# datasciencetoolkit/NextGP.jl

Measured on AMD Instinct MI355X. Metric: gibbs_iterations_per_sec, higher is better.
Workload: dtype f64; 1 GPU; single-trait Gibbs sweep, N=50000 individuals x P=600000 SNPs, marker sets BayesPR(200000) + BayesPR(200000) + BayesPR(200000), fp32 panel in HBM (BASELINE.json configs[3]: multi-breed random regression = three BayesPR marker sets of 200,000 SNPs); N=50000, P=600000, chains=1, panel_dtype=f32, accumulate_dtype=f64

## Files before the change

nextgp.jl_amd/csrc/ngp_api.hip:

```cpp
#include <hip/hip_runtime.h>

#include <dlfcn.h>

#include <algorithm>
#include <chrono>
#include <cmath>
#include <cstdio>
#include <cstdlib>
#include <condition_variable>
#include <cstddef>
#include <cstring>
#include <deque>
#include <memory>
#include <mutex>
#include <queue>
#include <string>
#include <thread>
#include <vector>

#include "../../include/nextgp_hip.h"
#include "ngp_kernels.h"
#include "ngp_random.h"
#include "ngp_dense.h"
#include "ngp_logvar.h"
// ... 25 lines not shown
    T *p = nullptr;
    PinnedArray() = default;
    PinnedArray(const PinnedArray &) = delete;
    PinnedArray &operator=(const PinnedArray &) = delete;
    PinnedArray(PinnedArray &&o) noexcept : p(o.p) { o.p = nullptr; }
    PinnedArray &operator=(PinnedArray &&o) noexcept { if (this != &o) { reset(); p = o.p; o.p = nullptr; } return *this; }
    ~PinnedArray() { reset(); }
    void reset() { if (p) { (void)hipHostFree(p); p = nullptr; } }
    hipError_t alloc_raw(size_t n) { reset(); const hipError_t e = hipHostMalloc((void **)&p, n * sizeof(T), hipHostMallocDefault); if (e != hipSuccess) p = nullptr; return e; }
    T *get() const { return p; }
    operator T *() const { return p; }
};

struct FileCloser {
    void operator()(FILE *f) const { std::fclose(f); }
};
using File = std::unique_ptr<FILE, FileCloser>;

struct HFix {
    int64_t ncol = 0, off = 0;
    DevArray<double> d_X, d_xpx0, d_xpxR, d_lhs0, d_rhs0;
};

struct DenseK {
    DevArray<double> K;
    int64_t q = 0, ld = 0;
    uint64_t digest = 0;
};

struct Grm {
    std::shared_ptr<DenseK> m;
    int state = 0, method = 1;
    int64_t N = 0, ncols = 0;
    double sum2pq = 0.0;
};

struct HRand {
    int64_t q = 0;
    double df = 0.0, scale = 0.0, varU0 = 0.0;
    bool offdiag = false;
    uint64_t fine_calls = 0;
    DevArray<long long> d_lptr, d_kptr;
    DevArray<int> d_lrows, d_level, d_kcol;
    DevArray<double> d_kval, d_kdiag, d_zpz;
    DevArray<double> d_u, d_sum_u;
    DevArray<double> d_vu;
    DevArray<double> d_scr;
    uint64_t sig = 0;
    std::shared_ptr<DenseK> dk;
    struct Launch { int wide; int d0, d1; long long r0, r1; };
    DevArray<int> d_order;
    DevArray<long long> d_dptr;
    std::vector<Launch> plan;
    int64_t ndepth = 0;
    int sched_mode = 0;
    bool scheduled() const { return sched_mode == 2 || (sched_mode == 0 && q > NGP_RS_AUTO_LEVELS_PER_DEPTH * ndepth); }
};

struct HLv {
    int set = -1;
    int64_t n = 0;
    int ncov = 0, mode = 0;
    double frac = 0.0, varZeta0 = 0.0;
    std::vector<double> zeta0;
    DevArray<double> d_C, d_iCpC, d_zeta, d_logv, d_part, d_vpart;
    DevArray<double> d_st;
    DevArray<int> d_trapseg;
};

struct PanelMem {
    DevArray<float> tiles;
    DevArray<double> mean;
    DevArray<double> gramx, mpm;
    double mpm_max = 0.0;
};

struct SampleStream {
    static constexpr int NSLOT = 4;
    File f;
    std::string path;
    size_t rec_bytes = 0;
    bool header_written = false;
    int device = 0;
    DevArray<unsigned char> d_slot[NSLOT];
    PinnedArray<unsigned char> h_slot[NSLOT];
    hipEvent_t ev_packed[NSLOT] = {nullptr, nullptr, nullptr, nullptr}, ev_copied[NSLOT] = {nullptr, nullptr, nullptr, nullptr};
    hipStream_t copy_stream = nullptr;
    std::thread writer;
    std::mutex mu;
    std::condition_variable cv;
    std::deque<int> queue;
    bool busy[NSLOT] = {false, false, false, false};
    bool stop = false, io_error = false;
    int64_t nenq = 0, nwritten = 0, ndropped = 0;
    ~SampleStream();
};

struct HSet {
    int64_t col0, ncol;
    int method;
    double df, scale;
    int64_t nreg;
    int64_t vb_off;
    int estPi;
    uint64_t fine_calls;
    double pi0;
    std::vector<double> vb0;
    int K = 0;
    std::vector<double> vcls, rpi;
    int tk = 0;
    int64_t nloc = 0;
    int lv = -1;
};

std::string g_create_err;


struct PlanRequest {
    int storage = 0;
    int mode = 1;
    int lag = 8;
    bool lag_auto = true;
    int near_req = 0;
    int max_shards_req = 0;
    int streamer_req = 0;
};

struct SweepPlan {
    int mode = 1;
    int64_t R = 0, S = 0;
    int V = 1;
    int D = 1;
    int NG = 1;
    int near = 3;
    int streamer = 1;
    int nchain = 8;
};

constexpr size_t NGP_LDS_MAX = 160 * 1024;

void choose_layout(int64_t N, int64_t max_shards, int64_t r_cap, int64_t *R, int64_t *S, bool prefer_odd = true) {
    int64_t r0 = (N + max_shards - 1) / max_shards;
    int64_t m = (r0 + 3) / 4;
    if (m < 1) m = 1;
    if (prefer_odd && (m & 1) == 0 && 4 * (m + 1) <= r_cap) m += 1;
    int64_t r = 4 * m;
    if (r > r_cap) r = r_cap;
    *R = r;
    *S = (N + r - 1) / r;
}

size_t sampler_lds(SweepKernel k) {
    const size_t base = (size_t)(3 * 4096 + 2 * NGP_RING * NGP_BLK + 6 * NGP_BLK) * sizeof(double) + 2 * NGP_BLK * sizeof(int) + 320;
    if (k == SweepKernel::lean) return base;
    if (k == SweepKernel::r || k == SweepKernel::multi_r) return base + NGP_SAMPLER_TUPLE_LDS + NGP_SAMPLER_R_LDS;
    return base + NGP_SAMPLER_TUPLE_LDS;
}

size_t streamer_lds(const SweepPlan &p, int K) {
    const int R = (int)p.R;
    if (K > 1) return p.streamer == 3 ? ngp_rows_multi_lds_bytes(R, K, true) : (p.streamer == 2 ? ngp_rows_multi_lds_bytes(R, K) : ngp_multi_lds_bytes(R, K));
    if (p.streamer >= 2) {
        const size_t nq = (p.streamer == 3) ? (size_t)R / 16 : (size_t)R / 4, hq = std::min<size_t>(NGP_ROWS_HMAX, (nq + 1) / 2);
        return (2 * nq + hq) * NGP_QS + (size_t)p.V * ((R + 7) & ~7) * 8 + 2 * NGP_ROWS_NW * NGP_BLK * 8 + 2 * NGP_DLS * 8 + 16 * 8 + 64 + 1024;
    }
    return 2 * (size_t)(R / 4) * NGP_QS + (size_t)R * 16 + 4096 + 2 * 512 + 128 + 3072 + (size_t)R * 64;
}

size_t sweep_lds(const SweepPlan &p, SweepKernel k, int K = 1) {
    const size_t streamer = streamer_lds(p, K);
    size_t lds = std::max(streamer, sampler_lds(k));
    if (K == 1 && streamer + 8192 <= NGP_LDS_MAX) lds = std::max(lds, streamer + 8192);
    return lds;
}

int fused_pair(const SweepPlan &p, int K) { return (p.streamer == 1 && K >= NGP_PAIR_FROM) ? 1 : 0; }

int64_t sweep_grid(const SweepPlan &p, int K = 1) { return K + ngp_multi_reducers(K, p.NG, fused_pair(p, K)) + p.S / p.V; }

SweepKernel pick_kernel(const SweepPlan &p, int K, bool diag, bool tup, bool rset) {
    if (K > 1) {
        if (rset && sweep_lds(p, SweepKernel::multi_r, K) <= NGP_LDS_MAX) return SweepKernel::multi_r;
        return tup ? SweepKernel::multi_tup : SweepKernel::multi;
    }
    if (p.V > 1) return SweepKernel::tall;
    if (diag) return SweepKernel::diag;
    if (rset && sweep_lds(p, SweepKernel::r) <= NGP_LDS_MAX) return SweepKernel::r;
    if (tup || rset) return SweepKernel::tup;
    return SweepKernel::lean;
}

const void *sweep_kernel(SweepKernel k) {
    for (auto unit : {sweep_kernel_0, sweep_kernel_1, sweep_kernel_2, sweep_kernel_3})
        if (const void *f = unit(k)) return f;
    return nullptr;
}

void launch_sweep_kernel(SweepKernel k, int64_t grid, size_t lds, hipStream_t stream, void *args) {
    void *a[] = {args};
    (void)hipLaunchKernel(sweep_kernel(k), dim3((unsigned)grid), dim3(NGP_WG), a, lds, stream);
}

int plan_sweep(int64_t N, int cu_count, const PlanRequest &q, SweepPlan *out, const char **msg) {
    SweepPlan p;
    p.mode = q.mode;
    int64_t max_shards = cu_count - 1 - (cu_count + NGP_GRP - 1) / NGP_GRP;
    if (q.max_shards_req > 0) max_shards = std::min<int64_t>(max_shards, q.max_shards_req);
    if (q.storage == 1) {
        if (q.mode != 1) { *msg = "compact storage runs in the persistent sweep (ngp_configure mode 1) only"; return NGP_ERR_ARG; }
        const int64_t r0 = (N + max_shards - 1) / max_shards;
        p.R = 16 * std::max<int64_t>(1, (r0 + 15) / 16);
        if (p.R > NGP_U8_MAX_R) { *msg = "N too large for one resident wave of streamers in compact storage"; return NGP_ERR_ARG; }
        p.S = (N + p.R - 1) / p.R;
        p.streamer = 3;
        p.nchain = NGP_ROWS_NW;
        const int nt = ngp_u8_tasks((int)p.R);
        const int want = q.lag_auto ? 8 : q.lag;
        if (nt == 1) p.D = want >= 12 ? 12 : (want >= 8 ? 8 : (want >= 6 ? 6 : (want >= 4 ? 4 : 3)));
        else if (nt == 2) p.D = want >= 8 ? 8 : 4;
        else p.D = 4;
        p.near = q.near_req ? q.near_req : ((p.R > 128) ? 2 : 3);
    } else {
        if (p.mode == 1) {
            int tallV = 0;
            int64_t w_max = 0;
            for (int v = 2; v <= 3 && !tallV; v++) {
                if (q.streamer_req != 0 && q.streamer_req != 2 * v) continue;
                if (q.streamer_req == 0 && N <= max_shards * 256) continue;
                SweepPlan t;
                t.V = v;
                auto fits = [&](int64_t w) { t.S = v * w; t.NG = (int)((t.S + NGP_GRP - 1) / NGP_GRP); return sweep_grid(t) <= cu_count; };
                int64_t w = cu_count - 1;
                while (w > 1 && !fits(w)) w--;
                if (q.max_shards_req > 0) w = std::max<int64_t>(1, std::min<int64_t>(w, q.max_shards_req / v));
                if (N <= v * w * NGP_ROWS_MAX_R && q.lag >= 3) { tallV = v; w_max = w; }
            }
            if (tallV) {
                choose_layout(N, tallV * w_max, NGP_ROWS_MAX_R, &p.R, &p.S, q.max_shards_req <= 0);
                p.S = (p.S + tallV - 1) / tallV * tallV;
                p.V = tallV;
            } else if (N > max_shards * 256) p.mode = 0;
            else choose_layout(N, max_shards, 256, &p.R, &p.S, q.max_shards_req <= 0);
        }
        if (p.mode == 0) choose_layout(N, 256, 508, &p.R, &p.S);
        p.D = (p.mode == 1) ? std::min(q.lag, 8) : 1;
        if (p.mode == 1 && p.R <= NGP_ROWS_MAX_R && q.lag >= 3 && (q.streamer_req == 2 || (q.streamer_req == 0 && p.R >= 64))) p.streamer = 2;
        if (p.V > 1) p.streamer = 2;
        p.nchain = (p.streamer == 2) ? NGP_ROWS_NW : 8;
        if (p.streamer == 2) {
            if (p.D > 6) p.D = 6;
            if (p.V > 1) p.D = (p.V == 2) ? 3 : 2;
        } else if (p.mode == 1 && p.R > 128 && p.D > 5) p.D = 5;
        else if (p.mode == 1 && q.lag_auto && p.D > 6) p.D = 6;
        p.near = q.near_req ? q.near_req : ((p.mode == 1 && p.streamer == 2 && p.R >= 64) ? 2 : ((p.mode == 1 && p.R > 128) ? 4 : 3));
    }
    p.NG = (int)((p.S + NGP_GRP - 1) / NGP_GRP);
    if (p.mode == 1) {
        if (!(p.NG <= 8 || p.D <= 3)) { *msg = "internal: more shard groups than the sampler adds"; return NGP_ERR_STATE; }
        if (sweep_lds(p, SweepKernel::tup) > NGP_LDS_MAX) { *msg = "panel too tall for the persistent sweep (LDS)"; return NGP_ERR_ARG; }
    }
    *out = p;
    return NGP_OK;
}

struct ChainMem {
    DevArray<double> d_lhs0, d_rhs0, d_beta, d_c, d_w, d_q, d_T, d_chi;
    DevArray<int8_t> d_setof;
    DevArray<int32_t> d_loc, d_vbidx;
    DevArray<uint8_t> d_delta;
    DevArray<double> d_sum_beta, d_sum_beta2, d_sum_delta;
    DevArray<double> d_ycorr, d_part, d_dlt;
    DevArray<double> d_rs;
    DevArray<DSet> d_sets;
    DevArray<DScal> d_scal;
    DevArray<double> d_cdlt;
    DevArray<unsigned long long> d_cdltg;
    DevArray<unsigned> d_ccnt;
    size_t ccnt_words = 0;
    size_t census_off = 0;
    unsigned long long *d_census_tbl = nullptr;
    DevArray<unsigned> abort_mem;
    unsigned *d_abort = nullptr;
    DevArray<double> d_tinv;
    int64_t tinv_blocks = 0;
    DevArray<unsigned> d_blin;
    int blin_for = -2;
    int lin_all = 0, lin_any = 0;
};

struct ModelMem {
    DevArray<double> d_varBeta, d_sum_varBeta;
    int64_t vb_cap = 0;
    DevArray<double> d_rcls;
    DevArray<DReg> d_regs;
    DevArray<long long> d_seg_k0;
    DevArray<int32_t> d_seg_len;
    DevArray<int32_t> d_seg_set;
    DevArray<double> d_segpart, d_regchi;
    DevArray<DTup> d_tup;
    DevArray<double> d_tupc, d_tupg, d_tsegpart;
    DevArray<DTReg> d_tregs;
    DevArray<long long> d_tseg_l0;
    DevArray<int32_t> d_tseg_len, d_tseg_set;
    std::vector<HFix> fix;
    int64_t nfixcol = 0;
    DevArray<double> d_bfix, d_sum_bfix;
    std::vector<HRand> rnd;
    std::vector<HLv> lv;
    DevArray<int64_t> d_trace_loci;
// ... 3617 lines not shown
```

nextgp.jl_amd/csrc/ngp_sweep.h:

```cpp
#pragma once
#include <cstddef>
#include <type_traits>
#include "ngp_sweep_args.h"

#ifndef NGP_ROWS_DPP
#define NGP_ROWS_DPP 1
#endif

#pragma clang fp contract(off)

namespace ngp {


#define NGP_DBG_FOLD                                                     \
    unsigned long long *const dbg = DBG ? A.dbg : nullptr;               \
    const int dbg_mode = DBG ? A.dbg_mode : 0;                           \
    (void)dbg; (void)dbg_mode;
#define NGP_DBG_LOCALS                                                   \
    unsigned long long *const dbg = A.dbg;                               \
    const int dbg_mode = A.dbg_mode;                                     \
    (void)dbg; (void)dbg_mode;
#define NGP_DBG_ROWS NGP_DBG_FOLD

__device__ inline unsigned ld_u32(const unsigned *p) { return __hip_atomic_load(p, __ATOMIC_RELAXED, __HIP_MEMORY_SCOPE_AGENT); }
// ... 1198 lines not shown
            return false;
        }
        __builtin_amdgcn_s_sleep(2);
    }
}

template <bool DBG>
__device__ __attribute__((always_inline)) inline void publish_block(const SweepArgs &A, int up, int j, const double *hist, const double *outb, const int *outi,
                                     const int *smeth, const double *ssdf) {
    NGP_DBG_LOCALS
    const int pbuf = up & 1;
    (void)hist;
    const long long k = (long long)(A.t0 + up) * NGP_BLK + j;
    const int si = A.setof[k];
    const double chik = A.chi[k];
    const int vbi = A.vbidx[k];
    st_f64(&A.dlt[(size_t)(up % NGP_RING) * NGP_BLK + j], hist[(up % NGP_RING) * NGP_BLK + j]);
    drain_vm();
    if (j == 0) st_u32(A.flag_dlt, (unsigned)(up + 1));
    if (dbg && j == 0) dbg[4 * (size_t)up + 2] = wall_clock64();
    const double bn = outb[pbuf * NGP_BLK + j];
    const int isave = outi[pbuf * NGP_BLK + j];
    A.beta[k] = bn;
    A.delta[k] = (uint8_t)isave;
    const int meth = (si >= 0) ? smeth[si] : -1;
    if (meth == 1) {
        double vb = 0.0;
        if (isave) {
            double tt = ssdf[si];
            double b2 = bn * bn;
            tt = tt + b2;
            vb = tt / chik;
            atomicAdd(&A.sets[si].nloci, 1);
        }
        A.varBeta[vbi] = vb;
    } else if (meth == 2) {
        if (isave) atomicAdd(&A.sets[si].nloci, 1);
    } else if (meth == 3) {
        atomicAdd(&A.sets[si].ncls[isave - 1], 1);
    }
}

struct RWide { double dmine; int c; };
__device__ __attribute__((noinline)) RWide rform_search_wide(const double *rcls, const size_t Ppad, const size_t col, const int j, const int Kk,
                                                             const double qv, const double av, const double tv, const double uv,
                                                             const double hs_k, const double rhs_k, const double bo_k) {
    const bool on = j < Kk;
    double q2 = qv, a2 = av, t2 = tv, u2 = uv;
    if (j >= NGP_RLDS && on) {
        const double *gp = rcls + (size_t)j * Ppad + col;
        const size_t gstr = (size_t)NGP_RMAX * Ppad;
        q2 = gp[0]; a2 = gp[gstr]; t2 = gp[2 * gstr]; u2 = gp[3 * gstr];
    }
    const double Lv = (q2 == 0.0) ? a2 : __builtin_fma(hs_k, q2, a2);
    RWide out;
    out.dmine = (q2 != 0.0) ? __builtin_fma(rhs_k, q2, t2) - bo_k : -bo_k;
    double m = readlane_d(Lv, 0);
#pragma unroll 1
    for (int v = 1; v < Kk; v++) {
        const double Lu = readlane_d(Lv, v);
        m = (Lu > m) ? Lu : m;
    }
    const double ev = on ? det_exp(Lv - m) : 0.0;
    double S = 0.0;
#pragma unroll 1
    for (int v = 0; v < Kk; v++) S = S + readlane_d(ev, v);
    int c = Kk - 1;
    double cum = 0.0;
#pragma unroll 1
    for (int v = 0; v < Kk; v++) {
        cum = cum + readlane_d(ev, v);
        const double thr = readlane_d(u2, v) * S;
        if (cum >= thr) { c = v; break; }
    }
    out.c = c;
    return out;
}

template <bool DBG, bool NGBIG = false, bool TUP = true, int RCLS = 1>
__device__ __attribute__((always_inline)) inline void role_sampler(const SweepArgs &A, char *smem) {
    NGP_DBG_LOCALS
    const int D = A.D, tid = threadIdx.x, wv = tid >> 6, j = tid & 63;
    double *Gd = (double *)smem;
    double *hist = Gd + 3 * 4096;
    double *vacc = hist + NGP_RING * NGP_BLK;
    double *r0 = vacc + NGP_RING * NGP_BLK;
    double *outb = r0 + 4 * NGP_BLK;
    int *outi = (int *)(outb + 2 * NGP_BLK);
    int *sabort = outi + 2 * NGP_BLK;
    int *totflag = sabort + 1;
    int *smeth = sabort + 4;
    double *ssdf = (double *)(sabort + 20);
    const int nb = A.t1 - A.t0;
    const size_t bsz = NGP_BLK * NGP_BLK;
    int *sK = sabort + 52;
    double *tl = (double *)(sabort + 80);
    int *tmeta = (int *)(tl + 2 * 9 * NGP_BLK);
    auto tuple_prefetch = [&](const int ub) __attribute__((always_inline)) {
        if (!TUP || !A.tup || ub >= nb) return;
        const long long tblk = (long long)(A.t0 + ub);
        const long long kcol = tblk * NGP_BLK + j;
        const int si = A.setof[kcol];
        const unsigned long long mask = __ballot(si >= 0 && smeth[si < 0 ? 0 : si] == NGP_METHOD_TUPLE_DEV);
        int *meta = tmeta + (ub & 1) * 4;
        if (mask == 0ull) {
            if (j == 0) meta[0] = 0;
            return;
        }
        const int sit = __builtin_amdgcn_readfirstlane(__shfl(si, __builtin_ctzll(mask)));
        const TupLane TL = load_tuplane(A.tupc, A.tupg, A.w, A.Ppad, kcol);
        const int k = A.tup[sit].k;
        const long long first_locus = (tblk - (A.tup[sit].col0 >> 6)) * tuple_loci_per_block(k);
        const int nvalid = tuple_nvalid(k, A.tup[sit].nloc, first_locus);
        double *dst = tl + (size_t)(ub & 1) * (9 * NGP_BLK) + j;
#pragma unroll
        for (int b = 0; b < NGP_KMAX; b++) { dst[b * NGP_BLK] = TL.crow[b]; dst[(NGP_KMAX + b) * NGP_BLK] = TL.grow[b]; }
        dst[2 * NGP_KMAX * NGP_BLK] = TL.ww;
        if (j == 0) { meta[0] = k; meta[1] = nvalid; }
    };
    double *rl = (double *)(tmeta + 16);
    int *rlm = (int *)(rl + 2 * 17 * NGP_BLK);
    int *rmeta = rlm + 2 * 128;
    double *rlx = (double *)(rmeta + 16);
    auto rcls_prefetch = [&](const int ub) __attribute__((always_inline)) {
        if (RCLS != 2 || !A.rcls || ub >= nb) return;
        const long long kcol = (long long)(A.t0 + ub) * NGP_BLK + j;
        const int si = A.setof[kcol];
        const int meth = (si >= 0) ? smeth[si] : -1;
        const int Kc = (si >= 0) ? sK[si] : 2;
        const unsigned long long mask = __ballot(meth == 3);
        if (j == 0) rmeta[(ub & 1) * 4] = (mask != 0ull) ? 1 : 0;
        if (mask == 0ull) return;
        RLane RL = empty_rlane();
        if (meth == 3) RL = load_rlane(A.rcls, A.Ppad, kcol, Kc, A.rhs0);
        double *dst = rl + (size_t)(ub & 1) * (17 * NGP_BLK) + j;
#pragma unroll
        for (int v = 0; v < NGP_RREG; v++) {
            dst[v * NGP_BLK] = RL.q[v]; dst[(4 + v) * NGP_BLK] = RL.a[v]; dst[(8 + v) * NGP_BLK] = RL.t[v]; dst[(12 + v) * NGP_BLK] = RL.u[v];
        }
        dst[16 * NGP_BLK] = RL.rhs0;
        rlm[(ub & 1) * 128 + j] = meth;
        rlm[(ub & 1) * 128 + 64 + j] = Kc;
        if (__ballot(meth == 3 && Kc > NGP_RREG) != 0ull) {
            double *dx = rlx + (size_t)(ub & 1) * (16 * NGP_BLK) + j;
#pragma unroll
            for (int arr = 0; arr < 4; arr++)
#pragma unroll
                for (int v = NGP_RREG; v < NGP_RLDS; v++) {
                    const bool on = (meth == 3) && v < Kc;
                    dx[(arr * 4 + v - NGP_RREG) * NGP_BLK] = on ? A.rcls[((size_t)arr * NGP_RMAX + v) * (size_t)A.Ppad + (size_t)kcol] : 0.0;
                }
        }
    };
    if (tid < 16) {
        smeth[tid] = A.sets[tid].method;
        ssdf[tid] = A.sets[tid].sdf;
        sK[tid] = A.sets[tid].K;
    }
    if (tid == 0) {
        *sabort = 0;
        *totflag = 0;
        st_u32(A.xcc_w, xcc_id() + 1u);
        if (dbg) { dbg[NGP_DBG_ALL - 2] = xcc_id(); dbg[NGP_DBG_ALL - 1] = (unsigned)__builtin_amdgcn_s_getreg((31 << 11) | 4); }
    }
    {
        const double *gd = chain_block_src(A, A.t0, A.lin_all || (A.blin && A.blin[A.t0] != 0u));
        for (int idx = tid; idx < 4096; idx += NGP_WG) Gd[idx] = gd[idx];
        if (nb > 1) {
            const double *gd1 = chain_block_src(A, A.t0 + 1, A.lin_all || (A.blin && A.blin[A.t0 + 1] != 0u));
            for (int idx = tid; idx < 4096; idx += NGP_WG) Gd[4096 + idx] = gd1[idx];
        }
    }
    __syncthreads();
    if (wv == 2) {
        double tot;
        if (fetch_group_sums<DBG, NGBIG>(A, 0, j, &tot)) r0[j] = tot;
        else if (j == 0) *sabort = 1;
    }
    if (wv == 1) { tuple_prefetch(0); rcls_prefetch(0); }
    __syncthreads();
    if (*sabort) return;
#define NGP_END_OF_BLOCK()                                                                       \
    do {                                                                                         \
        if (dbg && j == 0) dbg[NGP_DBG_WAVES + 8 * (size_t)u + wv] = wall_clock64();           \
        wg_barrier();                                                                            \
        if (*sabort) return;                                                                     \
    } while (0)
    if (wv == 0) {
        CoefRegs cur = load_coef(A, (long long)A.t0 * NGP_BLK + j), nxt = cur;
        double iVarE_sweep = 0.0;
        if constexpr (RCLS == 2) {
            if (A.rcls) iVarE_sweep = A.scal->iVarE;
        }
        for (int u = 0; u < nb; ++u) {
            const int t = A.t0 + u, buf = u & 1, slot = u % NGP_RING, rs = u & 3;
            if (dbg && j == 0) dbg[4 * (size_t)u] = wall_clock64();
            if (u + 1 < nb) nxt = load_coef(A, (long long)(t + 1) * NGP_BLK + j);
            constexpr bool PRELOAD = false;
            const bool tform = __builtin_amdgcn_readfirstlane((int)cur.tf) != 0;
            const double *gdb = Gd + (u % 3) * 4096 + j;
            double G[NGP_BLK];
            double tot;
            if (D == 1) {
                tot = r0[rs * NGP_BLK + j];
                bool okc = true;
                if (u >= 1) okc = fetch_group_sums<DBG, NGBIG>(A, u, j, &tot);
                if (!okc && j == 0) *sabort = 1;
            } else {
                for (unsigned sp = 0; lds_flag_ld(totflag) != u + 1; ++sp) {
                    if ((sp & 255u) == 255u && (lds_flag_ld(sabort) != 0 || sp > (NGP_SPIN_LIMIT << 4))) {
                        if (j == 0) *sabort = 1;
                        break;
                    }
                    __builtin_amdgcn_s_sleep(0);
                }
                asm volatile("" ::: "memory");
                tot = r0[rs * NGP_BLK + j];
            }
            if (DBG && dbg && j == 0) dbg[NGP_DBG_W5 + 4 * (size_t)u + 2] = wall_clock64();
            const double bo = cur.bo, cc = cur.cc, ww = cur.ww, st = cur.st;
            const double r = __builtin_fma(cur.gd, bo, tot);
#define NGP_LOAD_G()                                                           \
    if constexpr (!PRELOAD) { _Pragma("unroll") for (int kk = 0; kk < NGP_BLK; kk++) G[kk] = gdb[kk * NGP_BLK]; } \
    double H0 = -(cc * G[0]), H1 = -(cc * G[1]), H2 = -(cc * G[2]), H3 = -(cc * G[3]);
            double e = __builtin_fma(r, cc, ww);
            double dsave;
            int isave = 1;
            int meth0 = -1, si0 = -1, rblk = 0;
            if constexpr (RCLS == 1) {
                if (A.rcls) {
                    si0 = A.setof[(long long)t * NGP_BLK + j];
                    meth0 = (si0 >= 0) ? smeth[si0] : -1;
                }
            } else if constexpr (RCLS == 2) {
                if (A.rcls) rblk = __builtin_amdgcn_readfirstlane(rmeta[buf * 4]);
                if (rblk) meth0 = rlm[buf * 128 + j];
            }
            int tk = 0;
            if constexpr (TUP) {
                if (A.tup) tk = __builtin_amdgcn_readfirstlane(tmeta[buf * 4]);
            }
            if (tform && dbg_mode != 5) {
                double e0 = e;
                if constexpr (TUP) {
                    if (tk != 0) {
                        const int nvalid = __builtin_amdgcn_readfirstlane(tmeta[buf * 4 + 1]);
                        const double *tsrc = tl + (size_t)buf * (9 * NGP_BLK) + j;
                        TupLane TL;
#pragma unroll
                        for (int b = 0; b < NGP_KMAX; b++) { TL.crow[b] = tsrc[b * NGP_BLK]; TL.grow[b] = tsrc[(NGP_KMAX + b) * NGP_BLK]; }
                        TL.ww = tsrc[2 * NGP_KMAX * NGP_BLK];
                        e0 = tuple_e0(tk, nvalid, j, tot, bo, TL);
                    }
                }
                r0[rs * NGP_BLK + j] = e0;
                typedef const __attribute__((address_space(3))) double *lds_cdp;
                const lds_cdp ek = (lds_cdp)(r0 + rs * NGP_BLK);
                double s0 = 0.0, s1 = 0.0, s2 = 0.0, s3 = 0.0;
#pragma unroll
                for (int kk = 0; kk < NGP_BLK; kk += 16) {
                    double ev[16], tv[16];
#pragma unroll
                    for (int i = 0; i < 16; i++) ev[i] = ek[kk + i];
#pragma unroll
                    for (int i = 0; i < 16; i++) tv[i] = PRELOAD ? G[kk + i] : gdb[(kk + i) * NGP_BLK];
#pragma unroll
                    for (int i = 0; i < 16; i += 4) {
                        s0 = __builtin_fma(tv[i + 0], ev[i + 0], s0);
                        s1 = __builtin_fma(tv[i + 1], ev[i + 1], s1);
                        s2 = __builtin_fma(tv[i + 2], ev[i + 2], s2);
                        s3 = __builtin_fma(tv[i + 3], ev[i + 3], s3);
                    }
                    asm volatile("" : "+v"(s0), "+v"(s1), "+v"(s2), "+v"(s3));
                }
                dsave = (s0 + s1) + (s2 + s3);
                isave = 1;
            } else if (TUP && tk != 0) {
                const int nvalid = __builtin_amdgcn_readfirstlane(tmeta[buf * 4 + 1]);
                const double *tsrc = tl + (size_t)buf * (9 * NGP_BLK) + j;
                TupLane TL;
#pragma unroll
                for (int b = 0; b < NGP_KMAX; b++) { TL.crow[b] = tsrc[b * NGP_BLK]; TL.grow[b] = tsrc[(NGP_KMAX + b) * NGP_BLK]; }
                TL.ww = tsrc[2 * NGP_KMAX * NGP_BLK];
                dsave = tuple_chain_nv(tk, nvalid, j, tot, bo, TL, [&](int sl, int cc2) { return Gd[(u % 3) * 4096 + sl * NGP_BLK + cc2]; });
                isave = 1;
            } else if (RCLS != 0 && A.rcls && (RCLS == 2 ? rblk != 0 : __ballot(meth0 == 3) != 0ull)) {
                double dfin = 0.0;
                int cfin = 1;
                if constexpr (RCLS == 2) {
                    const double *cq = rl + (size_t)buf * (17 * NGP_BLK);
                    const double *cx = rlx + (size_t)buf * (16 * NGP_BLK);
                    const bool isr = (meth0 == 3);
                    const double q0j = cq[j], hstar = (isr && q0j == 0.0) ? cq[8 * NGP_BLK + j] : -1.0;
                    const double rhs0j = cq[16 * NGP_BLK + j];
                    const int Kj = rlm[buf * 128 + 64 + j];
                    const double iVarE = iVarE_sweep;
                    const int vj = (j < NGP_RLDS) ? j : 0;
                    const double *cls_base = (vj < NGP_RREG) ? cq + vj * NGP_BLK : cx + (vj - NGP_RREG) * NGP_BLK;
                    double rcur = r;
                    int kstart = 0;
                    for (int guard = 0; guard < NGP_BLK + 1; ++guard) {
                        double lazy_d, rhs = 0.0, hs = 0.0;
                        int lazy_c;
                        bool need;
                        if (isr) {
                            const double tt = rcur * iVarE;
                            rhs = tt + rhs0j;
                            const double s2 = rhs * rhs;
                            hs = 0.5 * s2;
                            need = (bo != 0.0) || !(hs <= hstar);
                            lazy_d = -bo;
                            lazy_c = 1;
                        } else {
                            eval_rform_other(rcur, bo, cc, ww, st, lazy_d, lazy_c);
                            need = (lazy_d != 0.0);
                        }
                        if (j >= kstart) { dfin = lazy_d; cfin = lazy_c; }
                        const unsigned long long todo = __ballot(need) & (~0ull << kstart);
                        if (!todo) break;
                        const int kk = __builtin_ctzll(todo);
                        const double Hk = -(gdb[kk * NGP_BLK]);
                        double dk;
                        if (__builtin_amdgcn_readlane(meth0, kk) == 3) {
                            const double rhs_k = readlane_d(rhs, kk), hs_k = readlane_d(hs, kk), bo_k = readlane_d(bo, kk);
                            const int Kk = __builtin_amdgcn_readlane(Kj, kk);
                            const bool on = j < Kk;
                            const double *cp = cls_base + kk;
                            const double qv = cp[0], av = cp[4 * NGP_BLK], tv = cp[8 * NGP_BLK], uv = cp[12 * NGP_BLK];
                            const double Lraw = (qv == 0.0) ? av : __builtin_fma(hs_k, qv, av);
                            const double dcls = __builtin_fma(rhs_k, qv, tv);
                            double dmine = (qv != 0.0) ? dcls - bo_k : -bo_k;
                            int c;
                            if (Kk <= NGP_RREG) {
                                const double Lv = on ? Lraw : -__builtin_inf();
                                const double up = on ? uv : __builtin_inf();
                                double m = __builtin_fmax(Lv, dpp_quad_f64<0xB1>(Lv));
                                m = __builtin_fmax(m, dpp_quad_f64<0x4E>(m));
                                const double ev = det_exp_le0(Lv - m);
                                const double c0 = dpp_quad_f64<0x00>(ev);
                                const double c1 = c0 + dpp_quad_f64<0x55>(ev);
                                const double c2 = c1 + dpp_quad_f64<0xAA>(ev);
                                const double c3 = c2 + dpp_quad_f64<0xFF>(ev);
                                const int vq = j & 3;
                                const double mycum = (vq == 0) ? c0 : ((vq == 1) ? c1 : ((vq == 2) ? c2 : c3));
                                const double thr = up * c3;
                                const unsigned hitm = (unsigned)__ballot(mycum >= thr) & 0xFu;
                                c = hitm ? __builtin_ctz(hitm) : Kk - 1;
                            } else if (Kk <= NGP_RLDS) {
                                const double Lv = Lraw;
                                double m = readlane_d(Lv, 0);
#pragma unroll
                                for (int v = 1; v < NGP_RLDS; v++) {
                                    if (v < Kk) {
                                        const double Lu = readlane_d(Lv, v);
                                        m = (Lu > m) ? Lu : m;
                                    }
                                }
                                const double ev = on ? det_exp(Lv - m) : 0.0;
                                double S = 0.0;
#pragma unroll
                                for (int v = 0; v < NGP_RLDS; v++)
                                    if (v < Kk) S = S + readlane_d(ev, v);
                                c = Kk - 1;
                                double cum = 0.0;
                                bool found = false;
#pragma unroll
                                for (int v = 0; v < NGP_RLDS; v++) {
                                    if (v < Kk && !found) {
                                        cum = cum + readlane_d(ev, v);
                                        const double thr = readlane_d(uv, v) * S;
                                        if (cum >= thr) { c = v; found = true; }
                                    }
                                }
                            } else {
                                const RWide rw = rform_search_wide(A.rcls, (size_t)A.Ppad, (size_t)((long long)t * NGP_BLK + kk), j, Kk, qv, av, tv, uv, hs_k, rhs_k, bo_k);
                                c = rw.c;
                                dmine = rw.dmine;
                            }
                            dk = readlane_d(dmine, c);
                            if (j == kk) { dfin = dk; cfin = c + 1; }
                        } else {
                            dk = readlane_d(lazy_d, kk);
                        }
                        if (dk != 0.0) rcur = __builtin_fma(Hk, dk, rcur);
                        kstart = kk + 1;
                        if (kstart >= NGP_BLK) break;
                    }
                } else {
                RLane RL = empty_rlane();
                double iVarE;
                {
                    if (meth0 == 3) RL = load_rlane(A.rcls, A.Ppad, (long long)t * NGP_BLK + j, sK[si0], A.rhs0);
                    iVarE = A.scal->iVarE;
                }
                double rcur = r;
                int kstart = 0;
                for (int guard = 0; guard < NGP_BLK + 1; ++guard) {
                    double cand;
                    int cls;
                    eval_rform(meth0, rcur, bo, cc, ww, st, RL, iVarE, cand, cls);
                    if (j >= kstart) { dfin = cand; cfin = cls; }
                    const unsigned long long todo = __ballot(cand != 0.0) & (~0ull << kstart);
                    if (!todo) break;
                    const int kk = __builtin_ctzll(todo);
                    const double dk = readlane_d(cand, kk);
                    const double Hk = -(gdb[kk * NGP_BLK]);
                    rcur = __builtin_fma(Hk, dk, rcur);
                    kstart = kk + 1;
                    if (kstart >= NGP_BLK) break;
                }
                }
                dsave = dfin;
                isave = cfin;
            } else if (dbg_mode == 5 && __ballot(st >= 0.0) == 0ull) {
                dsave = e;
            } else if (__ballot(st >= 0.0) == 0ull) {
                NGP_LOAD_G()
                if (DBG && dbg) {
                    asm volatile("s_waitcnt lgkmcnt(0)" ::: "memory");
                    if (j == 0) dbg[NGP_DBG_W5 + 4 * (size_t)u + 3] = wall_clock64();
                }
#pragma unroll
                for (int kk = 0; kk < NGP_BLK; kk += 4) {
                    double dk;
                    dk = readlane_d(e, kk + 0); e = __builtin_fma(H0, dk, e); H0 = -(cc * G[(kk + 4) & 63]);
                    dk = readlane_d(e, kk + 1); e = __builtin_fma(H1, dk, e); H1 = -(cc * G[(kk + 5) & 63]);
                    dk = readlane_d(e, kk + 2); e = __builtin_fma(H2, dk, e); H2 = -(cc * G[(kk + 6) & 63]);
                    dk = readlane_d(e, kk + 3); e = __builtin_fma(H3, dk, e); H3 = -(cc * G[(kk + 7) & 63]);
                }
                dsave = e;
            } else if (__popcll(__ballot((__builtin_fabs(r * cc) > st) || (bo != 0.0))) <= NGP_SPARSE_MAX) {
                double f = r * cc;
                const double nbo = -bo;
                unsigned long long todo = __ballot((__builtin_fabs(f) > st) || (bo != 0.0));
                while (todo) {
                    const int k = __builtin_ctzll(todo);
                    const double Hk = -(cc * gdb[k * NGP_BLK]);
                    const unsigned long long inm = __ballot(__builtin_fabs(f) > st);
                    const double ek = readlane_d(e, k), nk = readlane_d(nbo, k);
                    const double dk = ((inm >> k) & 1ull) ? ek : nk;
                    e = __builtin_fma(Hk, dk, e);
                    f = __builtin_fma(Hk, dk, f);
                    const unsigned long long later = (k == 63) ? 0ull : (~0ull << (k + 1));
                    todo = __ballot((__builtin_fabs(f) > st) || (bo != 0.0)) & later;
                }
                isave = __builtin_fabs(f) > st;
                dsave = isave ? e : -bo;
            } else {
                NGP_LOAD_G()
                double f = r * cc;
#pragma unroll
                for (int kk = 0; kk < NGP_BLK; kk += 4) {
#define NGP_STEP(HX, KO)                                              \
    {                                                                 \
        int in = __builtin_fabs(f) > st;                              \
        double dlv = in ? e : -bo;                                    \
        double dk = readlane_d(dlv, kk + KO);                         \
        e = __builtin_fma(HX, dk, e);                                 \
        f = __builtin_fma(HX, dk, f);                                 \
        HX = -(cc * G[(kk + KO + 4) & 63]);                           \
    }
                    NGP_STEP(H0, 0) NGP_STEP(H1, 1) NGP_STEP(H2, 2) NGP_STEP(H3, 3)
#undef NGP_STEP
                }
                isave = __builtin_fabs(f) > st;
                dsave = isave ? e : -bo;
            }
#undef NGP_LOAD_G
            hist[slot * NGP_BLK + j] = dsave;
            publish_dlt_granules(A.dltg, A.nonce, u, j, dsave);
            outb[buf * NGP_BLK + j] = bo + dsave;
            outi[buf * NGP_BLK + j] = isave;
            if (dbg && j == 0) dbg[4 * (size_t)u + 1] = wall_clock64();
            cur = nxt;
            NGP_END_OF_BLOCK();
        }
    } else if (wv == 1) {
        for (int u = 0; u < nb; ++u) {
            tuple_prefetch(u + 1);
            rcls_prefetch(u + 1);
            if (u >= 1) publish_block<DBG>(A, u - 1, j, hist, outb, outi, smeth, ssdf);
            NGP_END_OF_BLOCK();
        }
        if (nb >= 1) publish_block<DBG>(A, nb - 1, j, hist, outb, outi, smeth, ssdf);
    } else if (wv == 2) {
        if (D >= 4) {
            const double fxi = A.scal->fx_inv;
            unsigned long long qa = 0ull;
            int la = -1;
            int next_take = 1;
            if (nb > 1) {
                double tot1;
                if (fetch_group_sums<DBG, NGBIG>(A, 1, j, &tot1)) { r0[NGP_BLK + j] = tot1; next_take = 2; }
                else if (j == 0) *sabort = 1;
            }
            if (nb > 2) { qa = acc_load(A, 2, j); la = 2; }
            for (int u = 0; u < nb; ++u) {
                unsigned long long qn = 0ull;
                int ln = -1;
                {
                    const int want = (la >= 0 ? la : next_take - 1) + 1;
                    if (want < nb && want <= u + 3) { qn = acc_load(A, want, j); ln = want; }
                }
                if (next_take < nb && next_take <= u + 2) {
                    const bool must = (next_take == u + 1);
                    const unsigned terms = acc_terms(A, next_take);
                    unsigned long long q = qa;
                    bool ready = false;
                    int ok = 1;
                    if (la == next_take) ready = dbg_mode == 2 || acc_complete(q, terms);
                    else if (must || la < 0) { q = acc_load(A, next_take, j); ready = dbg_mode == 2 || acc_complete(q, terms); }
                    if (!ready && must) {
                        for (unsigned spins = 0;; ++spins) {
                            __builtin_amdgcn_s_sleep(2);
                            q = acc_load(A, next_take, j);
                            if (acc_complete(q, terms)) { ready = true; break; }
                            if ((spins & 7u) == 7u && ld_u32(A.abort_w) != 0u) { ok = 0; break; }
                            if (spins > (NGP_SPIN_LIMIT >> 3)) { st_u32(A.abort_w, 3u); ok = 0; break; }
                        }
                    }
                    if (!ok) {
                        if (j == 0) *sabort = 1;
                    } else if (ready) {
                        r0[(next_take & 3) * NGP_BLK + j] = acc_take(A, next_take, j, q, fxi);
                        if (dbg && j == 0) dbg[4 * (size_t)next_take + 3] = wall_clock64();
                        ++next_take;
                    }
                }
                if (ln == next_take) { qa = qn; la = ln; }
                else if (ln > next_take && ln >= 0) {
                    la = -1;
                    if (next_take < nb && next_take <= u + 3) { qa = acc_load(A, next_take, j); la = next_take; }
                } else la = -1;
                NGP_END_OF_BLOCK();
            }
        } else {
            for (int u = 0; u < nb; ++u) {
                if (u + 1 < nb && D >= 2) {
                    double tot;
                    if (fetch_group_sums<DBG, NGBIG>(A, u + 1, j, &tot)) r0[((u + 1) & 3) * NGP_BLK + j] = tot;
                    else if (j == 0) *sabort = 1;
                }
                NGP_END_OF_BLOCK();
            }
        }
    } else if (wv == 3) {
        const bool per_block = !A.lin_all && A.blin != nullptr;
        unsigned lin2 = A.lin_all ? 1u : 0u;
        if (per_block && nb > 2) lin2 = sld_u32(A.blin + A.t0 + 2);
        for (int u = 0; u < nb; ++u) {
            if (u + 2 < nb) {
                const char *gsrc = (const char *)chain_block_src(A, A.t0 + u + 2, lin2 != 0u) + (size_t)j * 16;
                char *gdst = (char *)(Gd + ((u + 2) % 3) * 4096);
#pragma unroll
                for (int i = 0; i < 32; i++)
                    __builtin_amdgcn_global_load_lds((const __attribute__((address_space(1))) void *)(gsrc + (size_t)i * 1024),
                                                     (__attribute__((address_space(3))) void *)(gdst + i * 1024), 16, 0, 0);
                asm volatile("s_waitcnt vmcnt(32)" ::: "memory");
            } else {
                drain_vm();
            }
            if (dbg && j == 0) dbg[NGP_DBG_WAVES + 8 * (size_t)u + wv] = wall_clock64();
            wg_barrier();
            unsigned ab;
            if (per_block && u + 3 < nb) sld_u32x2(A.abort_w, A.blin + A.t0 + u + 3, ab, lin2);
            else ab = sld_u32(A.abort_w);
            if (ab != 0u) return;
        }
    } else if (wv == 5) {
        double gxr[NGP_BLK];
#pragma unroll
        for (int kk = 0; kk < NGP_BLK; kk++) gxr[kk] = 0.0;
        for (int u = 0; u < nb; ++u) {
            if (D >= 2) {
                const int slot = u % NGP_RING, rs = u & 3;
                double tot = r0[rs * NGP_BLK + j];
                const bool have_far = (D >= 3) && (u >= 2) && (A.near >= 2);
                const bool have_one = (u >= 1);
                double cor = have_far ? vacc[slot * NGP_BLK + j] : 0.0;
                if (DBG && dbg) {
                    asm volatile("s_waitcnt vmcnt(0)" ::: "memory");
                    if (j == 0) dbg[NGP_DBG_W5 + 4 * (size_t)u] = wall_clock64();
                }
                if (have_one) {
                    typedef const __attribute__((address_space(3))) double *lds_cdp;
                    const lds_cdp dk = (lds_cdp)(hist + ((u - 1) % NGP_RING) * NGP_BLK);
                    double s0 = 0.0, s1 = 0.0, s2 = 0.0, s3 = 0.0;
#pragma unroll
                    for (int kk = 0; kk < NGP_BLK; kk += 16) {
                        double dv[16];
#pragma unroll
                        for (int i = 0; i < 16; i++) dv[i] = dk[kk + i];
#pragma unroll
                        for (int i = 0; i < 16; i += 4) {
                            s0 = __builtin_fma(gxr[kk + i + 0], dv[i + 0], s0);
                            s1 = __builtin_fma(gxr[kk + i + 1], dv[i + 1], s1);
                            s2 = __builtin_fma(gxr[kk + i + 2], dv[i + 2], s2);
                            s3 = __builtin_fma(gxr[kk + i + 3], dv[i + 3], s3);
                        }
                        asm volatile("" : "+v"(s0), "+v"(s1), "+v"(s2), "+v"(s3));
                    }
                    const double v1 = (s0 + s1) + (s2 + s3);
                    cor = have_far ? cor + v1 : v1;
                }
                if (have_far || have_one) tot = tot - cor;
                if (DBG && dbg && j == 0) dbg[NGP_DBG_W5 + 4 * (size_t)u + 1] = wall_clock64();
                r0[rs * NGP_BLK + j] = tot;
                asm volatile("s_waitcnt lgkmcnt(0)" ::: "memory");
                if (j == 0) lds_flag_st(totflag, u + 1);
                if (u + 1 < nb) {
                    load_rows_pair(A.gramx + ((size_t)(A.t0 + u + 1) * D + 1) * bsz, j, gxr);
                }
            }
            NGP_END_OF_BLOCK();
        }
    } else {
        const int fx = (wv == 4 && A.near >= 2) ? 2 : ((wv == 6 && A.near >= 3) ? 3 : (wv == 7 && A.near >= 4 ? 4 : 99));
        const int top = min(A.near, D - 1);
        double gr[NGP_BLK];
#pragma unroll
        for (int kk = 0; kk < NGP_BLK; kk++) gr[kk] = 0.0;
        bool have = false;
        for (int u = 0; u < nb; ++u) {
            if (fx < D) {
                if (u >= 1 && have) {
                    const int a = u - 1, upb = a + fx;
                    const double *dp = hist + (a % NGP_RING) * NGP_BLK;
                    double v = gemv4([&](int kk) { return gr[kk]; }, dp);
                    double *va = vacc + (upb % NGP_RING) * NGP_BLK + j;
                    const bool first = (fx == top) || (a == 0);
                    *va = first ? v : *va + v;
                }
                have = (u + fx < nb) && (u + 1 < nb);
                if (have) {
                    load_rows_pair(A.gramx + ((size_t)(A.t0 + u + fx) * D + fx) * bsz, j, gr);
                }
            }
            NGP_END_OF_BLOCK();
        }
    }
#undef NGP_END_OF_BLOCK
}

__device__ __attribute__((always_inline)) inline bool sweep_census(const SweepArgs &A, const int b, char *smem) {
    if (!A.census) return true;
    int *cflag = (int *)smem;
    if (threadIdx.x == 0) {
        A.census_tbl[b] = ((unsigned long long)(xcc_id() + 1u) << 32) | (unsigned)__builtin_amdgcn_s_getreg((31 << 11) | 4);
        if (A.census_fail != 0u && A.census_fail == A.iter_tag) atomicCAS(&A.census[1], 0u, 2u);
        const unsigned old = atomicAdd(&A.census[0], 1u);
        if (old + 1u == gridDim.x) atomicCAS(&A.census[1], 0u, 1u);
        const unsigned long long t0 = wall_clock64();
        unsigned verdict;
        while ((verdict = ld_u32(&A.census[1])) == 0u) {
            if (wall_clock64() - t0 > NGP_CENSUS_TICKS) atomicCAS(&A.census[1], 0u, 2u);
            else __builtin_amdgcn_s_sleep(8);
        }
        if (verdict != 1u) {
            st_u32(A.abort_w + 1, A.iter_tag);
            st_u32(A.abort_w, NGP_ABORT_CENSUS);
        }
        *cflag = (verdict == 1u) ? 1 : 0;
    }
    __syncthreads();
    const int cok = *cflag;
    __syncthreads();
    return cok != 0;
}

template <bool DBG>
__global__ __launch_bounds__(NGP_WG) __attribute__((amdgpu_waves_per_eu(2, 2))) void k_sweep(SweepArgs A) {
    constexpr bool TUP = DBG;
    constexpr int RCLSV = DBG ? 1 : 0;
#include "ngp_sweep_body.inc"
}
#if defined(NGP_INST_DBG) && NGP_INST_DBG == 2
__global__ __launch_bounds__(NGP_WG) __attribute__((amdgpu_waves_per_eu(2, 2))) void k_sweep_tup(SweepArgs A) {
    constexpr bool DBG = false, TUP = true;
    constexpr int RCLSV = 1;
#include "ngp_sweep_body.inc"
}
#endif
#if defined(NGP_INST_DBG) && NGP_INST_DBG == 3
__global__ __launch_bounds__(NGP_WG) __attribute__((amdgpu_waves_per_eu(2, 2))) void k_sweep_r(SweepArgs A) {
    constexpr bool DBG = false, TUP = true;
    constexpr int RCLSV = 2;
#include "ngp_sweep_body.inc"
}
#endif

// ... 661 lines not shown
```

nextgp.jl_amd/csrc/ngp_sweep_args.h:

```cpp
#pragma once
#include "ngp_common.h"

#define NGP_RING 16
#define NGP_MAX_LAG 12
#define NGP_SPIN_LIMIT (1u << 21)
#define NGP_WG 512
#define NGP_DBG_WAVES (1u << 19)
#define NGP_DBG_RED (3u << 18)
#define NGP_DBG_W5 (5u << 17)
#define NGP_DBG_ALL (7u << 17)
#define NGP_SPARSE_MAX 16
#ifndef NGP_LAZY_LAG
#define NGP_LAZY_LAG 7
#endif
#define NGP_QS 1040
#define NGP_SAMPLER_TUPLE_LDS (2 * 9 * 64 * 8 + 64)
#define NGP_SAMPLER_R_LDS (2 * 17 * 64 * 8 + 2 * 128 * 4 + 64 + 2 * 16 * 64 * 8)
#define NGP_ABORT_CENSUS 9u
#define NGP_CENSUS_TICKS 2000000ull
#define NGP_DBG_STREAM (1u << 20)

namespace ngp {

struct SweepArgs {
    const float *tiles;
    double *ycorr;
    const double *gramx;
    const double *tinv;
    const unsigned *blin;
    int lin_all;
    int knob;
    int variant;
    int V;
    int D, R, S, NG, near, fine_ok, t0, t1;
    double *beta;
    uint8_t *delta;
    const double *c, *w, *q, *mpm, *chi;
    const int8_t *setof;
    const int32_t *vbidx;
    DSet *sets;
    double *varBeta;
    const double *rcls;
    const double *rhs0;
    const DScal *scal;
    long long Ppad;
    const DTup *tup;
    const double *tupc, *tupg;
    const double *mean;
    long long N;
    unsigned long long *acc;
    double *dlt;
    unsigned long long *dltg;
    unsigned nonce;
    unsigned *flag_dlt;
    unsigned *abort_w;
    unsigned *census;
    unsigned long long *census_tbl;
    unsigned iter_tag;
    unsigned census_fail;
    unsigned *xcc_w;
    unsigned long long *dbg;
    int dbg_mode;
};

#define NGP_ROWS_MAX_R 224
#define NGP_ROWS_NW 7
#ifndef NGP_ROWS_HMAX
#define NGP_ROWS_HMAX 32
#endif
#define NGP_ROWS_PUBW 2
#define NGP_ROWS_POLLW 6
#define NGP_DLS 72

__host__ __device__ inline int ngp_u8_tasks(int R) {
    const int nuw = ((R >> 4) + NGP_ROWS_NW - 1) / NGP_ROWS_NW;
    const int nt = (4 * nuw + 7) / 8;
    return nt <= 1 ? 1 : (nt == 2 ? 2 : 4);
}
#define NGP_U8_MAX_R 896

#ifndef NGP_MAXC
#define NGP_MAXC 8
#endif
#ifndef NGP_PAIR_FROM
#define NGP_PAIR_FROM 4
#endif
__host__ __device__ inline int ngp_multi_reducers(int K, int NG, int pair) { return pair ? ((K + 1) / 2) * NG : K * NG; }
struct MultiArgs {
    int K, pair;
    SweepArgs a[NGP_MAXC];
};
struct ChainPtrs {
    double *ycorr;
    unsigned long long *acc;
    const double *dlt;
    const unsigned *flag_dlt;
};
__host__ __device__ inline size_t ngp_multi_chain_doubles(int R) { return (size_t)R + 512 + 128 + (size_t)8 * R; }
__host__ __device__ inline size_t ngp_multi_lds_bytes(int R, int K) {
    return (size_t)2 * (R >> 2) * NGP_QS + (size_t)K * ngp_multi_chain_doubles(R) * 8 + 64 + 3072;
}

__host__ __device__ inline size_t ngp_rows_multi_chain_doubles(int R) { return (size_t)((R + 7) & ~7) + 2 * NGP_ROWS_NW * NGP_BLK + 2 * NGP_DLS + 16; }
__host__ __device__ inline size_t ngp_rows_multi_lds_bytes(int R, int K, bool u8 = false) {
    const size_t nq = (size_t)R / (u8 ? 16 : 4), hq = nq + 1 < 2 * (size_t)NGP_ROWS_HMAX ? (nq + 1) / 2 : (size_t)NGP_ROWS_HMAX;
    return (2 * nq + hq) * NGP_QS + (size_t)K * ngp_rows_multi_chain_doubles(R) * 8 + 64 + 64 + 1024;
}

enum class SweepKernel { lean, diag, tup, r, tall, multi, multi_tup, multi_r };
const void *sweep_kernel_0(SweepKernel k);
const void *sweep_kernel_1(SweepKernel k);
const void *sweep_kernel_2(SweepKernel k);
const void *sweep_kernel_3(SweepKernel k);

}
```

Baseline: 42.26 it/s.

## Stage per-block coefficients through an LDS double buffer loaded by a helper wave

The sampler wave used to issue global loads for the next block's coefficients (bo, cc, ww, st, gd, tf) inside its serial per-block loop. Now wave 2 prefetches coefficients two blocks ahead and writes them into a two-slot LDS ring, and wave 0 reads the current block's coefficients from LDS. The aim is to take global-memory latency off the critical sampling path. The cost is extra LDS per workgroup (reusing the tuple/rl area) and reliance on the existing end-of-block barrier for ordering. It also adds a debug latch timestamp.

```diff
diff --git a/nextgp.jl_amd/csrc/ngp_api.hip b/nextgp.jl_amd/csrc/ngp_api.hip
--- a/nextgp.jl_amd/csrc/ngp_api.hip
+++ b/nextgp.jl_amd/csrc/ngp_api.hip
@@ -201,9 +201,9 @@
 
 size_t sampler_lds(SweepKernel k) {
     const size_t base = (size_t)(3 * 4096 + 2 * NGP_RING * NGP_BLK + 6 * NGP_BLK) * sizeof(double) + 2 * NGP_BLK * sizeof(int) + 320;
-    if (k == SweepKernel::lean) return base;
+    if (k == SweepKernel::lean) return base + NGP_SAMPLER_COEF_LDS;
     if (k == SweepKernel::r || k == SweepKernel::multi_r) return base + NGP_SAMPLER_TUPLE_LDS + NGP_SAMPLER_R_LDS;
-    return base + NGP_SAMPLER_TUPLE_LDS;
+    return base + NGP_SAMPLER_TUPLE_LDS + NGP_SAMPLER_COEF_LDS;
 }
 
 size_t streamer_lds(const SweepPlan &p, int K) {
diff --git a/nextgp.jl_amd/csrc/ngp_sweep.h b/nextgp.jl_amd/csrc/ngp_sweep.h
--- a/nextgp.jl_amd/csrc/ngp_sweep.h
+++ b/nextgp.jl_amd/csrc/ngp_sweep.h
@@ -1374,6 +1374,27 @@
                 }
         }
     };
+    constexpr bool STAGE = (NGP_COEF_STAGE != 0) && RCLS != 2;
+    char *cring = (char *)(TUP ? (void *)rl : (void *)tl);
+    auto coef_put = [&](const int ub, const CoefRegs &c) __attribute__((always_inline)) {
+        double *dst = (double *)(cring + (ub & 1) * NGP_COEF_SLOT);
+        dst[j] = c.bo; dst[NGP_BLK + j] = c.cc; dst[2 * NGP_BLK + j] = c.ww; dst[3 * NGP_BLK + j] = c.st; dst[4 * NGP_BLK + j] = c.gd;
+        if (j == 0) *(unsigned *)(dst + 5 * NGP_BLK) = c.tf;
+    };
+    auto coef_get = [&](const int ub) __attribute__((always_inline)) {
+        const double *src = (const double *)(cring + (ub & 1) * NGP_COEF_SLOT);
+        CoefRegs c;
+        c.bo = src[j]; c.cc = src[NGP_BLK + j]; c.ww = src[2 * NGP_BLK + j]; c.st = src[3 * NGP_BLK + j]; c.gd = src[4 * NGP_BLK + j];
+        c.tf = *(const unsigned *)(src + 5 * NGP_BLK);
+        return c;
+    };
+    CoefRegs cpend = {0.0, 0.0, 0.0, 0.0, 0.0, 0u};
+    auto coef_stage = [&](const int u) __attribute__((always_inline)) {
+        if constexpr (STAGE) {
+            if (u + 1 < nb) coef_put(u + 1, cpend);
+            if (u + 2 < nb) cpend = load_coef(A, (long long)(A.t0 + u + 2) * NGP_BLK + j);
+        }
+    };
     if (tid < 16) {
         smeth[tid] = A.sets[tid].method;
         ssdf[tid] = A.sets[tid].sdf;
@@ -1395,6 +1416,10 @@
     }
     __syncthreads();
     if (wv == 2) {
+        if constexpr (STAGE) {
+            coef_put(0, load_coef(A, (long long)A.t0 * NGP_BLK + j));
+            if (nb > 1) cpend = load_coef(A, (long long)(A.t0 + 1) * NGP_BLK + j);
+        }
         double tot;
         if (fetch_group_sums<DBG, NGBIG>(A, 0, j, &tot)) r0[j] = tot;
         else if (j == 0) *sabort = 1;
@@ -1409,7 +1434,8 @@
         if (*sabort) return;                                                                     \
     } while (0)
     if (wv == 0) {
-        CoefRegs cur = load_coef(A, (long long)A.t0 * NGP_BLK + j), nxt = cur;
+        CoefRegs cur = {0.0, 0.0, 0.0, 0.0, 0.0, 0u}, nxt = cur;
+        if constexpr (!STAGE) cur = nxt = load_coef(A, (long long)A.t0 * NGP_BLK + j);
         double iVarE_sweep = 0.0;
         if constexpr (RCLS == 2) {
             if (A.rcls) iVarE_sweep = A.scal->iVarE;
@@ -1417,7 +1443,8 @@
         for (int u = 0; u < nb; ++u) {
             const int t = A.t0 + u, buf = u & 1, slot = u % NGP_RING, rs = u & 3;
             if (dbg && j == 0) dbg[4 * (size_t)u] = wall_clock64();
-            if (u + 1 < nb) nxt = load_coef(A, (long long)(t + 1) * NGP_BLK + j);
+            if constexpr (STAGE) cur = coef_get(u);
+            else if (u + 1 < nb) nxt = load_coef(A, (long long)(t + 1) * NGP_BLK + j);
             constexpr bool PRELOAD = false;
             const bool tform = __builtin_amdgcn_readfirstlane((int)cur.tf) != 0;
             const double *gdb = Gd + (u % 3) * 4096 + j;
@@ -1694,8 +1721,17 @@
             outb[buf * NGP_BLK + j] = bo + dsave;
             outi[buf * NGP_BLK + j] = isave;
             if (dbg && j == 0) dbg[4 * (size_t)u + 1] = wall_clock64();
-            cur = nxt;
-            NGP_END_OF_BLOCK();
+            if constexpr (DBG) {
+                NGP_END_OF_BLOCK();
+                if (dbg && j == 0) dbg[NGP_DBG_LATCH + (size_t)u] = wall_clock64();
+                if constexpr (!STAGE) {
+                    asm volatile("" : "+v"(nxt.bo), "+v"(nxt.cc), "+v"(nxt.ww), "+v"(nxt.st), "+v"(nxt.gd), "+v"(nxt.tf) : : "memory");
+                    cur = nxt;
+                }
+            } else {
+                if constexpr (!STAGE) cur = nxt;
+                NGP_END_OF_BLOCK();
+            }
         }
     } else if (wv == 1) {
         for (int u = 0; u < nb; ++u) {
@@ -1718,6 +1754,7 @@
             }
             if (nb > 2) { qa = acc_load(A, 2, j); la = 2; }
             for (int u = 0; u < nb; ++u) {
+                coef_stage(u);
                 unsigned long long qn = 0ull;
                 int ln = -1;
                 {
@@ -1758,6 +1795,7 @@
             }
         } else {
             for (int u = 0; u < nb; ++u) {
+                coef_stage(u);
                 if (u + 1 < nb && D >= 2) {
                     double tot;
                     if (fetch_group_sums<DBG, NGBIG>(A, u + 1, j, &tot)) r0[((u + 1) & 3) * NGP_BLK + j] = tot;
diff --git a/nextgp.jl_amd/csrc/ngp_sweep_args.h b/nextgp.jl_amd/csrc/ngp_sweep_args.h
--- a/nextgp.jl_amd/csrc/ngp_sweep_args.h
+++ b/nextgp.jl_amd/csrc/ngp_sweep_args.h
@@ -9,6 +9,7 @@
 #define NGP_DBG_RED (3u << 18)
 #define NGP_DBG_W5 (5u << 17)
 #define NGP_DBG_ALL (7u << 17)
+#define NGP_DBG_LATCH ((3u << 18) + (1u << 16))
 #define NGP_SPARSE_MAX 16
 #ifndef NGP_LAZY_LAG
 #define NGP_LAZY_LAG 7
@@ -16,6 +17,11 @@
 #define NGP_QS 1040
 #define NGP_SAMPLER_TUPLE_LDS (2 * 9 * 64 * 8 + 64)
 #define NGP_SAMPLER_R_LDS (2 * 17 * 64 * 8 + 2 * 128 * 4 + 64 + 2 * 16 * 64 * 8)
+#ifndef NGP_COEF_STAGE
+#define NGP_COEF_STAGE 1
+#endif
+#define NGP_COEF_SLOT (5 * 64 * 8 + 8)
+#define NGP_SAMPLER_COEF_LDS (NGP_COEF_STAGE ? 2 * NGP_COEF_SLOT : 0)
 #define NGP_ABORT_CENSUS 9u
 #define NGP_CENSUS_TICKS 2000000ull
 #define NGP_DBG_STREAM (1u << 20)
```

Result: no change. 42.55 it/s, median of 4 (+0.7%).
